# wp133716/test_isaacgym

Measured on AMD Instinct MI355X. Metric: env-steps/sec (whole node), 4096 servo envs; 1/2/4/8-GPU scaling, higher is better.
Workload: dtype f32

## Files before the change

### test_isaacgym_amd/csrc/mg_internal.h

```cpp
#pragma once
#include <hip/hip_runtime.h>
#include <hip/hip_ext.h>
#include <stdint.h>
#include "../../include/migym.h"

#define MG_MAX_CONTACTS 8
#define MG_MAX_LINKS    32
#define MG_MAX_DOFS     32

struct MgStep {
    float h;
    float sub;
    float inv_sub;
    float inv_h;
    float inv_dt;
    float g[3];
    int   substeps, npos, nvel;
    float contact_offset, rest_offset, max_depen, bounce_thresh;
    int   has_ground;
    float n[3];
    float pd;
    float t1[3], t2[3];
    float mu_ground, e_ground;
    float fric_offset;
    float fric_corr;
};

#define MG_TREC_N        (MG_TBODY_F_N + MG_SHAPE_STRIDE + MG_MASS_N)
#define MG_TREC_MASS     (MG_TBODY_F_N + MG_SHAPE_STRIDE)
#ifndef MG_TREC_LDS_MAX
#define MG_TREC_LDS_MAX  (48 * 1024)
#endif

struct MgRigidArgs {
    int          nf;
    int          nf1;
    int          nb;
    const int*   free_ids;
    float*       state;
    const float* mass;
    const int*   body_tmpl;
    const float* tbf;
    const int*   tbi;
    const float* shapes;
    const float* hulls;
    const float* ext;
    float*       cforce;
    const float* trec;
    int          ntb;
    const float* root_src;
    const int*   root_row;
    float*       out_rb;
    float*       out_root;
    const int*   out_body;
    const int*   out_root_row;
    float*       gpatch;
    int          gstride;
    const int*   attr_idx;
    const float* attr;
};

struct MgArticArgs {
    int          na;
    int          nb, nd;
    const int*   artic_i;
    int          aff, ab0, ad0, ads;
    int          out_aff, og0, or0;
    int          tmpl;
    int          nl, ndof;
    int          nbl;
    int          fixed_base;
    int          chain;
    const float* link_f;
    const int*   link_i;
    float*       state;
    const float* mass;
    const int*   body_tmpl;
    const float* tbf;
    float*       dof_pos;
    float*       dof_vel;
    const float* dof_tpos;
    const float* dof_tvel;
    const float* dof_force;
    float*       tpos_w;
    float*       tvel_w;
    float*       force_w;
    const float* dof_props;
    const float* ext;
    float*       cforce;
    const float* uni;
    float*       out_rb;
    float*       out_root;
    float*       out_dof;
    const int*   out_body;
    const int*   out_root_row;
    const int*   attr_idx;
    const float* attr;
    float*       dof_frc;
};

#define MG_ENV_I_N    16
#define MG_ENV_G      16
#define MG_ENV_SLOTS_WIDE 32
#define MG_ENV_MAXF    2
#define MG_ENV_MAXS    4
#define MG_ENV_MAXCT  16
#define MG_ENV_MAXCT_WIDE 48
#define MG_ENV_FREE0  64
// ... 154 lines not shown
```

### test_isaacgym_amd/csrc/mg_rigid.hip

```cpp
#include "mg_internal.h"
#include "mg_math.h"
#include "mg_attractor.h"

#ifdef MG_RIGID1_STAMPS
#define MG_RIGID1_NSTAMP 18
__device__ unsigned long long g_rigid_stamp[4096][MG_RIGID1_NSTAMP];
extern "C" int mg_debug_rigid_stamps(unsigned long long* out, int nwaves) {
    if (nwaves > 4096) nwaves = 4096;
    return hipMemcpyFromSymbol(out, HIP_SYMBOL(g_rigid_stamp), (size_t)nwaves * MG_RIGID1_NSTAMP * 8) == hipSuccess
               ? 0
               : -1;
}
__device__ __forceinline__ unsigned long long rigid_stamp() {
    unsigned long long t;
    __builtin_amdgcn_sched_barrier(0);
    asm volatile("s_memtime %0\n\ts_waitcnt lgkmcnt(0)" : "=s"(t)::"memory");
    __builtin_amdgcn_sched_barrier(0);
    return t;
}
#define RSTAMP(k) do { const unsigned long long t_ = rigid_stamp(); \
    if (threadIdx.x == 0 && blockIdx.x < 4096) g_rigid_stamp[blockIdx.x][k] = t_; } while (0)
#define RUSE(v) asm volatile("" ::"v"(v))
#else
#define RSTAMP(k) do { } while (0)
// ... 523 lines not shown
                const float raw = fmaf(an[a].k2, (pos ? an[a].e2 : 0.0f) - v2, an[a].l2);
                const float nl = clamp_sym(raw, lim);
                const float dl = nl - an[a].l2;
                const bool cl = last && (raw > lim || raw < -lim);
                if (a == 0) c02 = cl; else c12 = cl;
                an[a].l2 = nl;
                V.x = fmaf(-dl, invm, V.x);
                W = pfma(pk2(an[a].I2.x, an[a].I2.y), bc2(dl), W);
                Z.x = fmaf(an[a].I2.z, dl, Z.x);
            }
        }
    };
    const f2 nsub = bc2(-P.inv_sub), psub = bc2(P.sub);
    const int nit = P.npos + P.nvel;
    for (int it = 0; it < P.npos; ++it) {
        const f2 t0 = sep(0) * nsub, t1 = sep(1) * nsub;
        const float tg[4] = {fminf(t0.x, P.max_depen), fminf(t0.y, P.max_depen), fminf(t1.x, P.max_depen),
                             fminf(t1.y, P.max_depen)};
        if (it == 0) {
#pragma unroll
            for (int j = 0; j < 4; ++j) normal(j, tg[j]);
        }
        anchors(true, it == nit - 1);
#pragma unroll
        for (int j = 0; j < 4; ++j) normal(j, tg[j]);
        DV = pfma(V, psub, DV);
        DW = pfma(W, psub, DW);
        DZ = pfma(Z, psub, DZ);
    }
    if (P.nvel > 0) {
        const f2 s01 = sep(0), s23 = sep(1);
        const float sj[4] = {s01.x, s01.y, s23.x, s23.y};
        float tg[4];
#pragma unroll
        for (int j = 0; j < 4; ++j) tg[j] = vel_target(P, sj[j], e, sl[j].vn0);
        for (int it = P.npos; it < nit; ++it) {
#pragma unroll
            for (int j = 0; j < 4; ++j) normal(j, tg[j]);
            anchors(false, it == nit - 1);
#pragma unroll
            for (int j = 0; j < 4; ++j) normal(j, tg[j]);
        }
    }
    v = v3(V.x, V.y, Z.y);
    w = v3(W.x, W.y, Z.x);
    dx = v3(DV.x, DV.y, DZ.y);
    dth = v3(DW.x, DW.y, DZ.x);
}

template <bool PACK, bool ATTR, class B>
__device__ __forceinline__ void rigid_body1(const B& G, const MgStep& P, const float* T, V3& x, Q4& q, V3& v,
                                            V3& w, V3& fsum, float invm, V3 invI, Q4 iq, V3 com, bool has_ext,
                                            V3 fext, V3 text, const float* hulls, float* gp, int gstride,
                                            const float* at) {
    const float lin_damp = T[0], ang_damp = T[1], max_lv = T[2], max_av = T[3], grav_on = T[4];
    float shr[MG_SHAPE_STRIDE];
    const float* sh = T + MG_TBODY_F_N;
    if constexpr (PACK && MG_RIGID1_SHAPE_REGS) {
#pragma unroll
        for (int k = 0; k < 14; ++k) shr[k] = sh[k];
        sh = shr;
    }
    const bool has_shape = P.has_ground && sh[0] >= 0.0f;
    const float rho = sh[13];
    const float h = P.h;
    const float lin_keep = 1.0f - fminf(lin_damp * h, 1.0f);
    const float ang_keep = 1.0f - fminf(ang_damp * h, 1.0f);
    const float max_lv2 = max_lv * max_lv;
    const float max_av2 = max_av * max_av;
    const float mu = 0.5f * (sh[11] + P.mu_ground);
    const float e = 0.5f * (sh[12] + P.e_ground);
    const V3 n0 = v3(P.n[0], P.n[1], P.n[2]);
    GPatch R;
    R.cnt = 0;
    R.dirty = false;
    R.nA = R.aA[0] = R.aA[1] = R.aB[0] = R.aB[1] = v3(0.0f, 0.0f, 0.0f);
    {
        const float clear = G.dn(x) + P.pd;
        const bool far = rho >= 0.0f && clear - rho > P.contact_offset + 1e-3f * (1.0f + fabsf(clear) + rho);
        if (gp && has_shape && !far) {
            float r[MG_FP_N];
#pragma unroll
            for (int k = 0; k < MG_FP_N; ++k) r[k] = gp[(size_t)k * gstride];
            R.cnt = (int)r[0];
            R.nA = v3(r[1], r[2], r[3]);
#pragma unroll
            for (int k = 0; k < 2; ++k) {
                R.aA[k] = v3(r[4 + 6 * k], r[5 + 6 * k], r[6 + 6 * k]);
                R.aB[k] = v3(r[7 + 6 * k], r[8 + 6 * k], r[9 + 6 * k]);
            }
        }
    }

    RUSE(R.cnt); RUSE(R.aA[1].z);
    RSTAMP(2);
    q = qnormalize(q);
    for (int st = 0; st < P.substeps; ++st) {
        const S3 Iw = sym_rdrt(qmat(inertia_frame(q, iq)), invI);
        const V3 xc = com_world(x, q, com);

        if (grav_on != 0.0f) v = vmad(v, v3(P.g[0], P.g[1], P.g[2]), h);
        if (has_ext) {
            v = vmad(v, fext, invm * h);
            w = vmad(w, symmul(Iw, text), h);
        }
        if constexpr (ATTR) {
            if (at) attr_free_body(at, x, q, xc, invm, invI, iq, h, v, w);
        }
        v = vscale(v, lin_keep);
        w = vscale(w, ang_keep);
        {
            float v2 = vdot(v, v);
            if (v2 > max_lv2) v = vscale(v, sqrtf(max_lv2 / v2));
            float w2 = vdot(w, w);
            if (w2 > max_av2) w = vscale(w, sqrtf(max_av2 / w2));
        }

        RUSE(v.x); RUSE(w.z); RUSE(xc.x);
        if (st < 2) RSTAMP(3 + 6 * st);
        NRow sl[4];
        bool on[4];
        V3 cp[4];
#pragma unroll
        for (int j = 0; j < 4; ++j) {
            on[j] = false;
            sl[j].r = v3(0.0f, 0.0f, 0.0f);
            sl[j].s0 = 0.0f;
            cp[j] = v3(0.0f, 0.0f, 0.0f);
        }
        const float clear = G.dn(x) + P.pd;
        const bool far = rho >= 0.0f && clear - rho > P.contact_offset + 1e-3f * (1.0f + fabsf(clear) + rho);
        if (__any(has_shape && !far) && has_shape)
            shape_candidates(G, P, sh, q, x, hulls, [&](int k, V3 p, float sep, float, float) {
// ... 90 lines not shown
                        an[a].l2 = nl;
                        v = G.f2(v, dl, invm);
                        w = fmad3(w, an[a].I2, dl);
                    }
                }
                normals();
                if (pos) {
                    dx = fmad3(dx, v, P.sub);
                    dth = fmad3(dth, w, P.sub);
                }
            }
#pragma unroll
            for (int j = 0; j < 4; ++j) fsum = G.addn(fsum, sl[j].ln);
#pragma unroll
            for (int a = 0; a < 2; ++a) {
                fsum = G.add1(fsum, an[a].l1);
                fsum = G.add2(fsum, an[a].l2);
            }
            const bool one = R.cnt < 2;
            if ((c01 && (c11 || one)) || (c02 && (c12 || one))) R.cnt = 0;
        } else {
            for (int it = 0; it < P.npos; ++it) {
                dx = fmad3(dx, v, P.sub);
                dth = fmad3(dth, w, P.sub);
            }
        }

        RUSE(dx.x); RUSE(dth.z);
        if (st < 2) RSTAMP(7 + 6 * st);
        const V3 xc1 = vadd(xc, dx);
        q = qintegrate(q, dth);
        x = origin_from_com(xc1, q, com);
        RUSE(x.x); RUSE(q.w);
        if (st < 2) RSTAMP(8 + 6 * st);
    }
    if (gp && has_shape) {
        gp[0] = (float)R.cnt;
        if (R.cnt > 0 && R.dirty) {
            const float r[MG_FP_N] = {0.0f, R.nA.x, R.nA.y, R.nA.z,
                                      R.aA[0].x, R.aA[0].y, R.aA[0].z, R.aB[0].x, R.aB[0].y, R.aB[0].z,
                                      R.aA[1].x, R.aA[1].y, R.aA[1].z, R.aB[1].x, R.aB[1].y, R.aB[1].z};
#pragma unroll
            for (int k = 1; k < MG_FP_N; ++k) gp[(size_t)k * gstride] = r[k];
        }
    }
}

#ifndef MG_RIGID1_ROUND_WAVES
#define MG_RIGID1_ROUND_WAVES 2
#endif
#ifndef MG_RIGID1_WIDE_WAVES
#define MG_RIGID1_WIDE_WAVES 3
#endif
template <bool UPZ, bool LDS_T, bool WIDE, bool ATTR>
__global__ void __launch_bounds__(64, UPZ && WIDE ? MG_RIGID1_WIDE_WAVES : (UPZ ? MG_RIGID1_ROUND_WAVES : 2))
k_rigid_step1(MgStep P, MgRigidArgs A) {
    extern __shared__ float s_trec[];
    const int i = (WIDE ? gridDim.x - 1 - blockIdx.x : blockIdx.x) * 64 + threadIdx.x;
    RSTAMP(0);
    const bool live = i < A.nf;
    const int b = A.free_ids ? A.free_ids[live ? i : A.nf - 1] : (live ? i : A.nf - 1);
    const int nb = A.nb;
    const float* Si = A.state + b;
    int si = nb;
    if (A.root_src) {
        const int rr = A.root_row[b];
        if (rr >= 0) {
            Si = A.root_src + (size_t)rr * MG_STATE_N;
            si = 1;
        }
    }
    V3 x = v3(Si[0 * si], Si[1 * si], Si[2 * si]);
    Q4 q = q4(Si[3 * si], Si[4 * si], Si[5 * si], Si[6 * si]);
    V3 v = v3(Si[7 * si], Si[8 * si], Si[9 * si]);
    V3 w = v3(Si[10 * si], Si[11 * si], Si[12 * si]);
    const int tb = A.body_tmpl[b];
#ifdef MG_RIGID1_PREFETCH_OUT
    const bool fout = (A.out_rb || A.out_root) && !WIDE;
    const int pre_ob = fout && A.out_rb ? A.out_body[b] : -1;
    const int pre_or = fout && A.out_root ? A.out_root_row[b] : -1;
#endif
    V3 fext = v3(0.0f, 0.0f, 0.0f), text = v3(0.0f, 0.0f, 0.0f);
    if (A.ext) {
        fext = v3(A.ext[0 * nb + b], A.ext[1 * nb + b], A.ext[2 * nb + b]);
        text = v3(A.ext[3 * nb + b], A.ext[4 * nb + b], A.ext[5 * nb + b]);
    }
    const float* T;
    if constexpr (LDS_T) {
        for (int k = threadIdx.x; k < A.ntb * MG_TREC_N; k += 64) s_trec[k] = A.trec[k];
        __syncthreads();
        T = s_trec + tb * MG_TREC_N;
    } else {
        T = A.trec + tb * MG_TREC_N;
    }
    float mr[11];
    if (T[5] != 0.0f) {
#pragma unroll
        for (int k = 0; k < 11; ++k) mr[k] = T[MG_TREC_MASS + k];
    } else {
#pragma unroll
        for (int k = 0; k < 11; ++k) mr[k] = A.mass[k * nb + b];
    }
    const float invm = mr[0];
    const V3 invI = v3(mr[1], mr[2], mr[3]);
    const Q4 iq = q4(mr[4], mr[5], mr[6], mr[7]);
    const V3 com = v3(mr[8], mr[9], mr[10]);
    V3 fsum = v3(0.0f, 0.0f, 0.0f);
    RUSE(x.x); RUSE(q.w); RUSE(w.z); RUSE(invm); RUSE(com.z); RUSE(T[4]);
    RSTAMP(1);
    float* gp = live && A.gpatch ? A.gpatch + b : nullptr;
    const float* at = nullptr;
    if constexpr (ATTR) {
        const int ai = A.attr_idx[b];
        if (live && ai >= 0) at = A.attr + (size_t)ai * MG_ATTR_N;
    }
    if constexpr (UPZ) {
        rigid_body1<!WIDE, ATTR>(BasisZ{}, P, T, x, q, v, w, fsum, invm, invI, iq, com, A.ext != nullptr, fext, text,
                                 A.hulls, gp, A.gstride, at);
    } else {
        BasisGen G;
        G.n = v3(P.n[0], P.n[1], P.n[2]);
        G.t1 = v3(P.t1[0], P.t1[1], P.t1[2]);
        G.t2 = v3(P.t2[0], P.t2[1], P.t2[2]);
        rigid_body1<!WIDE, ATTR>(G, P, T, x, q, v, w, fsum, invm, invI, iq, com, A.ext != nullptr, fext, text, A.hulls,
                                 gp, A.gstride, at);
    }
    int bo = b;
    asm volatile("" : "+v"(bo));
    if (live) {
        float* So = A.state;
        So[0 * nb + bo] = x.x; So[1 * nb + bo] = x.y; So[2 * nb + bo] = x.z;
        So[3 * nb + bo] = q.x; So[4 * nb + bo] = q.y; So[5 * nb + bo] = q.z; So[6 * nb + bo] = q.w;
        So[7 * nb + bo] = v.x; So[8 * nb + bo] = v.y; So[9 * nb + bo] = v.z;
        So[10 * nb + bo] = w.x; So[11 * nb + bo] = w.y; So[12 * nb + bo] = w.z;
        A.cforce[0 * nb + bo] = fsum.x * P.inv_dt;
        A.cforce[1 * nb + bo] = fsum.y * P.inv_dt;
        A.cforce[2 * nb + bo] = fsum.z * P.inv_dt;
    }
    if ((A.out_rb || A.out_root) && !WIDE) {
        if (live) {
            const float o[MG_STATE_N] = {x.x, x.y, x.z, q.x, q.y, q.z, q.w, v.x, v.y, v.z, w.x, w.y, w.z};
#ifdef MG_RIGID1_PREFETCH_OUT
            const int ob = pre_ob;
            const int rr = pre_or;
#else
            const int ob = A.out_rb ? A.out_body[bo] : -1;
            const int rr = A.out_root ? A.out_root_row[bo] : -1;
#endif
            if (A.out_rb) {
                float* R = A.out_rb + (size_t)ob * MG_STATE_N;
#pragma unroll
                for (int k = 0; k < MG_STATE_N; ++k) R[k] = o[k];
            }
            if (rr >= 0) {
                float* Ro = A.out_root + (size_t)rr * MG_STATE_N;
#pragma unroll
                for (int k = 0; k < MG_STATE_N; ++k) Ro[k] = o[k];
            }
        }
        RSTAMP(15);
#ifdef MG_RIGID1_STAMPS
        asm volatile("s_waitcnt vmcnt(0)" ::: "memory");
        RSTAMP(16);
#endif
    } else if (A.out_rb || A.out_root) {
        __shared__ float s_out[64 * 16];
        __shared__ int s_dst[2][64];
        const int l = threadIdx.x;
        const float o[MG_STATE_N] = {x.x, x.y, x.z, q.x, q.y, q.z, q.w, v.x, v.y, v.z, w.x, w.y, w.z};
#pragma unroll
        for (int k = 0; k < MG_STATE_N; ++k) s_out[l * 16 + k] = o[k];
        s_dst[0][l] = live && A.out_rb ? A.out_body[bo] : -1;
        s_dst[1][l] = live && A.out_root ? A.out_root_row[bo] : -1;
        __syncthreads();
#pragma unroll
        for (int k = 0; k < MG_STATE_N; ++k) {
            const int e = k * 64 + l;
            const int row = e / MG_STATE_N, col = e - row * MG_STATE_N;
            const float val = s_out[row * 16 + col];
            const int d0 = s_dst[0][row], d1 = s_dst[1][row];
            if (d0 >= 0) A.out_rb[(size_t)d0 * MG_STATE_N + col] = val;
            if (d1 >= 0) A.out_root[(size_t)d1 * MG_STATE_N + col] = val;
        }
    }
}

template <bool UPZ, int MAXC, bool MULTI, bool ATTR>
__global__ void __launch_bounds__(64) k_rigid_step(MgStep P, MgRigidArgs A) {
    const int i = blockIdx.x * 64 + threadIdx.x;
    if (i >= A.nf) return;
    const int b = A.free_ids ? A.free_ids[i] : i;
    if constexpr (UPZ) {
        rigid_body<MAXC, MULTI, ATTR>(BasisZ{}, P, A, b);
    } else {
        BasisGen G;
        G.n = v3(P.n[0], P.n[1], P.n[2]);
        G.t1 = v3(P.t1[0], P.t1[1], P.t1[2]);
        G.t2 = v3(P.t2[0], P.t2[1], P.t2[2]);
        rigid_body<MAXC, MULTI, ATTR>(G, P, A, b);
    }
}

}

bool mg_step_is_upz(const MgStep& P) {
    return P.n[0] == 0.0f && P.n[1] == 0.0f && P.n[2] == 1.0f && P.t1[0] == 0.0f && P.t1[1] == 1.0f &&
           P.t1[2] == 0.0f && P.t2[0] == -1.0f && P.t2[1] == 0.0f && P.t2[2] == 0.0f;
}

static int mg_cu_count() {
    static int cus[64] = {0};
    int dev = 0;
    if (hipGetDevice(&dev) != hipSuccess || dev < 0 || dev >= 64) return 256;
    if (cus[dev] <= 0) {
        int n = 0;
        if (hipDeviceGetAttribute(&n, hipDeviceAttributeMultiprocessorCount, dev) != hipSuccess || n <= 0) n = 256;
        cus[dev] = n;
    }
    return cus[dev];
}

hipError_t mg_launch_rigid_step(const MgStep& P, const MgRigidArgs& A, hipStream_t s) {
    if (A.nf <= 0) return hipSuccess;
    const bool upz = mg_step_is_upz(P);
    MgRigidArgs A1 = A, A2 = A;
    A2.root_src = nullptr;
    A2.out_rb = nullptr;
    A2.out_root = nullptr;
    A2.gpatch = nullptr;
    A1.nf = A.nf1;
    A2.nf = A.nf - A.nf1;
    if (A.free_ids) {
        A2.free_ids = A.free_ids + A.nf1;
    } else {
        A2.state = A.state + A.nf1;
        A2.mass = A.mass + A.nf1;
        A2.body_tmpl = A.body_tmpl + A.nf1;
        A2.ext = A.ext ? A.ext + A.nf1 : nullptr;
        A2.cforce = A.cforce + A.nf1;
        A2.attr_idx = A.attr_idx ? A.attr_idx + A.nf1 : nullptr;
    }
    if (A1.nf > 0) {
        const int blocks = (A1.nf + 63) / 64;
        const bool wide = blocks > mg_cu_count() * 4 * (upz ? MG_RIGID1_ROUND_WAVES : 2);
        const size_t lds = (size_t)A.ntb * MG_TREC_N * sizeof(float);
#define MG_K1(U, L) \
    do { \
        if (wide) MG_LAUNCH((k_rigid_step1<U, L, true, false>), dim3(blocks), dim3(64), L ? lds : 0, s, P, A1); \
        else MG_LAUNCH((k_rigid_step1<U, L, false, false>), dim3(blocks), dim3(64), L ? lds : 0, s, P, A1); \
    } while (0)
        if (A1.attr_idx) {
            if (upz && wide) MG_LAUNCH((k_rigid_step1<true, false, true, true>), dim3(blocks), dim3(64), 0, s, P, A1);
            else if (upz) MG_LAUNCH((k_rigid_step1<true, false, false, true>), dim3(blocks), dim3(64), 0, s, P, A1);
            else if (wide) MG_LAUNCH((k_rigid_step1<false, false, true, true>), dim3(blocks), dim3(64), 0, s, P, A1);
            else MG_LAUNCH((k_rigid_step1<false, false, false, true>), dim3(blocks), dim3(64), 0, s, P, A1);
        } else if (lds <= MG_TREC_LDS_MAX) {
            if (upz) MG_K1(true, true);
            else MG_K1(false, true);
        } else {
            if (upz) MG_K1(true, false);
            else MG_K1(false, false);
        }
#undef MG_K1
    }
    if (A2.nf > 0) {
        const int blocks = (A2.nf + 63) / 64;
        if (A2.attr_idx) {
            if (upz) MG_LAUNCH((k_rigid_step<true, MG_MAX_CONTACTS, true, true>), dim3(blocks), dim3(64), 0, s, P, A2);
            else MG_LAUNCH((k_rigid_step<false, MG_MAX_CONTACTS, true, true>), dim3(blocks), dim3(64), 0, s, P, A2);
        } else if (upz) MG_LAUNCH((k_rigid_step<true, MG_MAX_CONTACTS, true, false>), dim3(blocks), dim3(64), 0, s, P, A2);
        else MG_LAUNCH((k_rigid_step<false, MG_MAX_CONTACTS, true, false>), dim3(blocks), dim3(64), 0, s, P, A2);
    }
    return hipGetLastError();
}
```

### test_isaacgym_amd/csrc/migym_capi.cpp

```cpp
#include <hip/hip_runtime.h>

#include <algorithm>
#include <array>
#include <cmath>
#include <cstdio>
#include <cstdarg>
#include <cstring>
#include <string>
#include <map>
#include <vector>

#include "mg_internal.h"
#include "mg_chainlink.h"
#include "mg_attractor.h"

thread_local MgKernelTimer* mg_timer = nullptr;

namespace {

thread_local std::string g_err;

int fail(int code, const char* fmt, ...) __attribute__((format(printf, 2, 3)));
int fail(int code, const char* fmt, ...) {
    char buf[512];
// ... 41 lines not shown
    int attr_count = 0, plain_count = 0;
};

enum AttrClass : char { ATTR_NONE = 0, ATTR_FREE, ATTR_LINK, ATTR_ENV_LINK, ATTR_ENV_FREE, ATTR_PILE };

struct EnvGroup {
    int tmpl, first_link, nl, ndof, floating;
    int wide;
    int max_free;
    int offset, count;
};

}

struct mg_sim {
    int device = 0;
    mg_sim_params params{};
    bool uploaded = false;

    int nenv = 0, na = 0, nb = 0, nd = 0, ntb = 0, ns = 0, nf = 0, nartic = 0, ntl = 0;
    int max_actor_dofs = 0;
    int nf1 = 0;
    int nf_rigid = 0;

    float* d_state = nullptr;
    float* d_mass = nullptr;
    int* d_body_tmpl = nullptr;
    int* d_free_global = nullptr;
    int* d_perm = nullptr;
    float* d_tbf = nullptr;
    float* d_trec = nullptr;
    int* d_tbi = nullptr;
    float* d_shapes = nullptr;
    float* d_hulls = nullptr;
    float* d_shape_obb = nullptr;
    int* d_actor_root = nullptr;
    int* d_body_actor = nullptr;
    int* d_root_row = nullptr;
    bool roots_free = false;
    int fusion = 0;
    const float* pend_root = nullptr;
    const float* pend_tgt[3] = {nullptr, nullptr, nullptr};
    unsigned long long pend_root_cap = 0, pend_tgt_cap[3] = {0, 0, 0}, rb_cap = 0;
    float* bind_root = nullptr;
    float* bind_rb = nullptr;
    float* bind_dof = nullptr;
    long long state_gen = 0, rb_gen = -1, out_gen = -1;
    unsigned long long out_cap = 0;
    long long dof_sgen = 0, dof_gen = -1;
    unsigned long long dof_cap = 0;
    bool step_out_ok = false;
    int* d_slot_global = nullptr;
    int* d_slot_actor = nullptr;
    int last_set_deferred = 0;
    int* d_actor_dof = nullptr;
    float* d_cforce = nullptr;
    float* d_ext = nullptr;
    bool ext_pending = false;

    float* d_dof = nullptr;
    float* d_dof_tgt = nullptr;
    float* d_dof_props = nullptr;
    int* d_artic = nullptr;
    float* d_link_f = nullptr;
    int* d_link_i = nullptr;
    std::vector<ArticGroup> groups;
    int* d_artic_step = nullptr;
    int* d_env = nullptr;
    int* d_pairs = nullptr;
    float* d_fpatch = nullptr;
    float* d_gpatch = nullptr;
    float* d_chain_uni = nullptr;
    unsigned* d_fp_mask = nullptr;
    float* d_env_carry = nullptr;
    int nhull_floats = 0;
    float* d_env_ctab = nullptr;
    int n_coupled = 0;
    std::vector<EnvGroup> env_groups;
    int n_pile = 0;
    int* d_pile_i = nullptr;
    int* d_pile_body = nullptr;
    unsigned* d_pile_pairs = nullptr;
    int* d_pile_slots = nullptr;

    float* d_stage = nullptr;
    size_t stage_n = 0;
    char* h_pin = nullptr;
    size_t h_pin_n = 0;
    hipEvent_t pin_ev = nullptr;
    bool pin_ev_pending = false;
    float* d_host_out = nullptr;
    size_t host_out_n = 0;
    bool has_light = false;
    mg_light light{};
    float* h_stage = nullptr;
    float* d_stage_alias = nullptr;
    size_t h_stage_n = 0;
    float* h_root_in = nullptr;
    float* d_root_in_alias = nullptr;
    hipEvent_t root_ev = nullptr;
    bool root_ev_pending = false;
    bool ho_alias = false;
    const float* ho_written = nullptr;
    long long ho_root_gen = -1, ho_rb_gen = -1, ho_dof_gen = -1;
    int* d_stage_idx = nullptr;
    size_t stage_idx_n = 0;
// ... 187 lines not shown
    HIP_TRY(hipMemcpyAsync(s->d_dof_tgt + (size_t)k * s->nd, src, (size_t)s->nd * sizeof(float),
                           hipMemcpyDeviceToDevice, st));
    return MG_OK;
}

int set_dof_columns(mg_sim* s, const float* src, int src_host, int ncol, float* dst0, float* dst1,
                    const int* idx, int n_idx, hipStream_t st) {
    if (!s || !s->uploaded) return fail(MG_ERR_STATE, "sim has no uploaded model");
    if (s->nd == 0) return MG_OK;
    if (!src) return fail(MG_ERR_ARG, "null source tensor");
    if (idx && n_idx < 0) return fail(MG_ERR_ARG, "negative index count");
    HIP_TRY(hipSetDevice(s->device));
    const float* dsrc;
    const int* didx;
    int rc = stage_src(s, src, src_host, (size_t)s->nd * ncol, idx, n_idx, st, &dsrc, &didx);
    if (rc) return rc;
    float* dst[2] = {dst0, dst1};
    if (idx)
        HIP_TRY(mg_launch_scatter_dofs(dsrc, ncol, s->d_actor_dof, didx, n_idx, s->na, s->max_actor_dofs, dst, st));
    else
        HIP_TRY(mg_launch_scatter_dofs(dsrc, ncol, nullptr, nullptr, s->nd, 0, 1, dst, st));
    return MG_OK;
}

void shape_obb(const float* sh, const float* hulls, float* o) {
    const int t = (int)sh[0];
    for (int k = 0; k < MG_OBB_N; ++k) o[k] = 0.0f;
    if (t == MG_SHAPE_CONVEX && hulls) {
        const float* hv = hulls + (int)sh[2];
        const int nv = (int)hv[0];
        float lo[3], hi[3];
        for (int c = 0; c < 3; ++c) { lo[c] = hv[MG_HULL_HEADER + c]; hi[c] = lo[c]; }
        for (int i = 1; i < nv; ++i)
            for (int c = 0; c < 3; ++c) {
                const float v = hv[MG_HULL_HEADER + 3 * i + c];
                lo[c] = std::min(lo[c], v);
                hi[c] = std::max(hi[c], v);
            }
        for (int c = 0; c < 3; ++c) {
            o[c] = 0.5f * (lo[c] + hi[c]);
            o[3 + c] = 0.5f * (hi[c] - lo[c]);
        }
    } else if (t == MG_SHAPE_BOX) {
        o[3] = sh[1]; o[4] = sh[2]; o[5] = sh[3];
    } else if (t == MG_SHAPE_CAPSULE) {
        o[3] = sh[1] + sh[2]; o[4] = sh[1]; o[5] = sh[1];
    } else {
        o[3] = sh[1]; o[4] = sh[1]; o[5] = sh[1];
    }
}

void free_all(mg_sim* s) {
    void* ptrs[] = {s->d_state, s->d_mass, s->d_body_tmpl, s->d_free_global, s->d_perm, s->d_tbf, s->d_trec, s->d_tbi, s->d_shapes, s->d_hulls, s->d_shape_obb,
                    s->d_actor_root, s->d_root_row, s->d_slot_global, s->d_slot_actor, s->d_body_actor, s->d_actor_dof, s->d_cforce, s->d_ext, s->d_dof, s->d_dof_tgt, s->d_dof_frc,
                    s->d_dof_props, s->d_artic, s->d_artic_step, s->d_env, s->d_pairs, s->d_fpatch, s->d_gpatch, s->d_chain_uni, s->d_fp_mask, s->d_env_carry, s->d_env_ctab, s->d_link_f, s->d_link_i, s->d_stage, s->d_stage_idx, s->d_host_out,
                    s->d_pile_i, s->d_pile_body, s->d_pile_pairs, s->d_pile_slots, s->d_rstate, s->d_rshapes, s->d_env_shape_first, s->d_cams};
    for (void* p : ptrs)
        if (p) (void)hipFree(p);
}

}

extern "C" {

int32_t mg_abi_version(void) { return MG_ABI_VERSION; }
const char* mg_last_error(void) { return g_err.c_str(); }

int32_t mg_device_count(void) {
    int n = 0;
    if (hipGetDeviceCount(&n) != hipSuccess) return 0;
    return n;
}

mg_sim* mg_create_sim(int32_t device, const mg_sim_params* params) {
    if (!params) { fail(MG_ERR_ARG, "null params"); return nullptr; }
    int n = mg_device_count();
    if (n <= 0) { fail(MG_ERR_DEVICE, "no HIP device available (libmigym needs an MI355X)"); return nullptr; }
    if (device < 0 || device >= n) { fail(MG_ERR_DEVICE, "device %d out of range (%d visible)", device, n); return nullptr; }
    if (hipSetDevice(device) != hipSuccess) { fail(MG_ERR_DEVICE, "hipSetDevice(%d) failed", device); return nullptr; }
    mg_sim* s = new mg_sim();
    s->device = device;
    s->params = *params;
    for (int k = 0; k < mg_sim::kRing; ++k) {
        bool ok = hipEventCreate(&s->ring_b[k]) == hipSuccess && hipEventCreate(&s->ring_e[k]) == hipSuccess;
        for (int j = 0; j < mg_sim::kKern && ok; ++j)
            ok = hipEventCreate(&s->kern_b[k][j]) == hipSuccess && hipEventCreate(&s->kern_e[k][j]) == hipSuccess;
        if (!ok) {
            fail(MG_ERR_DEVICE, "hipEventCreate failed");
            mg_destroy_sim(s);
            return nullptr;
        }
    }
    return s;
}

void mg_destroy_sim(mg_sim* s) {
    if (!s) return;
    (void)hipSetDevice(s->device);
    (void)hipDeviceSynchronize();
    free_all(s);
    for (int k = 0; k < mg_sim::kRing; ++k) {
        if (s->ring_b[k]) (void)hipEventDestroy(s->ring_b[k]);
        if (s->ring_e[k]) (void)hipEventDestroy(s->ring_e[k]);
        for (int j = 0; j < mg_sim::kKern; ++j) {
            if (s->kern_b[k][j]) (void)hipEventDestroy(s->kern_b[k][j]);
            if (s->kern_e[k][j]) (void)hipEventDestroy(s->kern_e[k][j]);
        }
// ... 593 lines not shown
        std::vector<float> trec((size_t)s->ntb * MG_TREC_N, 0.0f);
        for (int t = 0; t < s->ntb; ++t) {
            float* r = &trec[(size_t)t * MG_TREC_N];
            std::memcpy(r, m->tmpl_body_f + (size_t)t * MG_TBODY_F_N, MG_TBODY_F_N * sizeof(float));
            const int s0 = m->tmpl_body_i[t * MG_TBODY_I_N + 0], sc = m->tmpl_body_i[t * MG_TBODY_I_N + 1];
            if (sc > 0) {
                const float* sr = m->shapes + (size_t)s0 * MG_SHAPE_STRIDE;
                std::memcpy(r + MG_TBODY_F_N, sr, MG_SHAPE_STRIDE * sizeof(float));
                double ext = -1.0;
                switch ((int)sr[0]) {
                    case MG_SHAPE_SPHERE: ext = sr[1]; break;
                    case MG_SHAPE_BOX: ext = std::sqrt((double)sr[1] * sr[1] + (double)sr[2] * sr[2] + (double)sr[3] * sr[3]); break;
                    case MG_SHAPE_CAPSULE: ext = (double)sr[1] + sr[2]; break;
                    case MG_SHAPE_CONVEX: ext = sr[1]; break;
                    default: break;
                }
                const double po = std::sqrt((double)sr[4] * sr[4] + (double)sr[5] * sr[5] + (double)sr[6] * sr[6]);
                r[MG_TBODY_F_N + 13] = (ext >= 0.0 && std::isfinite(ext + po)) ? (float)((ext + po) * (1.0 + 1e-6)) : -1.0f;
            } else {
                r[MG_TBODY_F_N] = -1.0f;
            }
        }
        std::vector<int> seen(s->ntb, 0), uniform(s->ntb, 1);
        for (int b = 0; b < nb; ++b) {
            if (m->body_kind[b] != MG_BODY_FREE) continue;
            const int t = m->body_tmpl[b];
            const float* mr = m->body_mass + (size_t)b * MG_MASS_N;
            float* r = &trec[(size_t)t * MG_TREC_N];
            if (!seen[t]) {
                std::memcpy(r + MG_TREC_MASS, mr, MG_MASS_N * sizeof(float));
                seen[t] = 1;
            } else if (std::memcmp(r + MG_TREC_MASS, mr, MG_MASS_N * sizeof(float)) != 0) {
                uniform[t] = 0;
            }
        }
        for (int t = 0; t < s->ntb; ++t) trec[(size_t)t * MG_TREC_N + 5] = seen[t] && uniform[t] ? 1.0f : 0.0f;
        HIP_TRY(h2d(s->d_trec, trec.data(), trec.size() * sizeof(float)));
    }
    HIP_TRY(h2d(s->d_shapes, m->shapes, (size_t)s->ns * MG_SHAPE_STRIDE * sizeof(float)));
    if (m->hulls) HIP_TRY(h2d(s->d_hulls, m->hulls, (size_t)m->num_hull_floats * sizeof(float)));
    {
        std::vector<float> obb((size_t)std::max(s->ns, 1) * MG_OBB_N, 0.0f);
        for (int k = 0; k < s->ns; ++k) shape_obb(m->shapes + (size_t)k * MG_SHAPE_STRIDE, m->hulls, &obb[(size_t)k * MG_OBB_N]);
        HIP_TRY(dalloc(&s->d_shape_obb, obb.size()));
        HIP_TRY(h2d(s->d_shape_obb, obb.data(), obb.size() * sizeof(float)));
    }
    HIP_TRY(h2d(s->d_actor_root, root_int.data(), (size_t)na * sizeof(int)));
    {
        std::vector<int> body_actor(nb, -1);
        for (int a = 0; a < na; ++a) body_actor[m->actor_root_body[a]] = a;
        HIP_TRY(dalloc(&s->d_body_actor, (size_t)std::max(nb, 1)));
        HIP_TRY(h2d(s->d_body_actor, body_actor.data(), (size_t)nb * sizeof(int)));
    }
    {
        std::vector<int> row(nb, -1);
        bool ok = s->nf1 == s->nf_rigid && s->nf_rigid == s->nf && s->nartic == 0 && s->n_coupled == 0 &&
                  s->n_pile == 0 && na > 0;
        for (int a = 0; a < na && ok; ++a) {
            const int slot = root_int[a];
            ok = slot >= 0 && slot < s->nf1 && row[slot] < 0;
            if (ok) row[slot] = a;
        }
        s->roots_free = ok;
        HIP_TRY(dalloc(&s->d_root_row, (size_t)std::max(nb, 1)));
        HIP_TRY(h2d(s->d_root_row, row.data(), (size_t)nb * sizeof(int)));
    }
    {
        std::vector<int> slot_actor(nb, -1);
        for (int a = 0; a < na; ++a) slot_actor[root_int[a]] = a;
        HIP_TRY(dalloc(&s->d_slot_global, (size_t)std::max(nb, 1)));
        HIP_TRY(h2d(s->d_slot_global, order.data(), (size_t)nb * sizeof(int)));
        HIP_TRY(dalloc(&s->d_slot_actor, (size_t)std::max(nb, 1)));
        HIP_TRY(h2d(s->d_slot_actor, slot_actor.data(), (size_t)nb * sizeof(int)));
        for (ArticGroup& g : s->groups) {
            g.out_aff = 0;
            if (!g.aff) continue;
            const int* r0 = artic_step.data() + (size_t)g.step_offset * MG_ARTIC_I_N;
            const int G0 = order[r0[0]], A0 = slot_actor[r0[0]];
            bool ok = A0 >= 0;
            for (int k = 0; k < g.step_count && ok; ++k) {
                const int* r = r0 + (size_t)k * MG_ARTIC_I_N;
                ok = slot_actor[r[0]] == A0 + k;
                for (int l = 0; l < g.nl && ok; ++l) ok = order[r[0] + l * r[3]] == G0 + k * g.nl + l;
            }
            if (ok) { g.out_aff = 1; g.out_g0 = G0; g.out_r0 = A0; }
        }
        long long covered = s->nf1 == s->nf_rigid && s->nf_rigid == s->nf ? s->nf1 : -1;
        for (const ArticGroup& g : s->groups) {
            if (covered < 0) break;
            if (g.count == 0) continue;
            if (!(g.chain && g.nl >= 2 && g.nl <= 4) || g.step_count != g.count) covered = -1;
            else covered += (long long)g.step_count * g.nbody;
        }
        s->step_out_ok = s->n_coupled == 0 && s->n_pile == 0 && nb > 0 && covered == nb;
    }
    HIP_TRY(h2d(s->d_actor_dof, m->actor_dof, (size_t)(na + 1) * sizeof(int)));
    HIP_TRY(hipMemset(s->d_cforce, 0, (size_t)nb * 3 * sizeof(float)));
    HIP_TRY(hipMemset(s->d_dof_frc, 0, std::max<size_t>((size_t)nd * 2, 1) * sizeof(float)));
    s->h_actor_dof.assign(m->actor_dof, m->actor_dof + (na > 0 ? na + 1 : 0));
    s->dof_frc_n = 0;
    HIP_TRY(hipMemset(s->d_ext, 0, (size_t)nb * 6 * sizeof(float)));
    if (nd > 0) {
        std::vector<float> ds = to_soa(m->dof_state0, nd, 2);
        HIP_TRY(h2d(s->d_dof, ds.data(), ds.size() * sizeof(float)));
        HIP_TRY(hipMemset(s->d_dof_tgt, 0, (size_t)nd * 3 * sizeof(float)));
        std::vector<float> dp = to_soa(m->dof_props, nd, MG_DOFPROP_N);
        HIP_TRY(h2d(s->d_dof_props, dp.data(), dp.size() * sizeof(float)));
    }
    for (ArticGroup& g : s->groups)
        if (g.uni_mass) chain_uni_dof(m->dof_props, g);
    HIP_TRY(dalloc(&s->d_chain_uni, std::max<size_t>(s->groups.size(), 1) * MG_CHAIN_UNI_N));
    HIP_TRY(chain_uni_upload(s));
    HIP_TRY(h2d(s->d_artic, artic_sorted.data(), artic_sorted.size() * sizeof(int)));
    HIP_TRY(h2d(s->d_artic_step, artic_step.data(), artic_step.size() * sizeof(int)));
    HIP_TRY(h2d(s->d_env, env_flat.data(), env_flat.size() * sizeof(int)));
    HIP_TRY(h2d(s->d_pairs, pairs.data(), pairs.size() * sizeof(int)));
    if (s->n_pile > 0) {
        std::vector<int> flat;
        for (const auto& r : pile_rows) flat.insert(flat.end(), r.begin(), r.end());
        HIP_TRY(dalloc(&s->d_pile_i, flat.size()));
        HIP_TRY(h2d(s->d_pile_i, flat.data(), flat.size() * sizeof(int)));
        HIP_TRY(dalloc(&s->d_pile_body, pile_body.size()));
        HIP_TRY(h2d(s->d_pile_body, pile_body.data(), pile_body.size() * sizeof(int)));
        HIP_TRY(dalloc(&s->d_pile_pairs, std::max<size_t>(pile_pairs.size(), 1)));
        if (!pile_pairs.empty())
            HIP_TRY(h2d(s->d_pile_pairs, pile_pairs.data(), pile_pairs.size() * sizeof(unsigned)));
// ... 133 lines not shown
        }
    }
    for (const EnvGroup& g : s->env_groups) {
        MgEnvArgs A{};
        A.ne = g.count; A.nb = s->nb; A.nd = s->nd;
        A.env_i = s->d_env + (size_t)g.offset * MG_ENV_I_N;
        A.pairs = s->d_pairs;
        A.fpatch = s->d_fpatch;
        A.fp_mask = s->d_fp_mask + (size_t)g.offset * MG_FP_W;
        A.carry = s->d_env_carry + (size_t)g.offset * mg_env_carry_floats();
        A.ctab = s->d_env_ctab + (size_t)g.offset * mg_env_ctab_floats();
        A.nl = g.tmpl >= 0 ? g.nl : 0;
        A.ndof = g.tmpl >= 0 ? g.ndof : 0;
        A.floating = g.tmpl >= 0 ? g.floating : 0;
        A.max_free = g.max_free;
        A.link_f = s->d_link_f + (size_t)(g.tmpl >= 0 ? g.first_link : 0) * MG_LINK_F_N;
        A.link_i = s->d_link_i + (size_t)(g.tmpl >= 0 ? g.first_link : 0) * MG_LINK_I_N;
        A.state = s->d_state; A.mass = s->d_mass; A.body_tmpl = s->d_body_tmpl;
        A.tbf = s->d_tbf; A.tbi = s->d_tbi; A.shapes = s->d_shapes; A.hulls = s->d_hulls;
        A.shape_obb = s->d_shape_obb;
        A.nhull = s->nhull_floats;
        A.nshape = s->ns;
        A.dof_pos = s->d_dof; A.dof_vel = s->d_dof + s->nd;
        A.dof_tpos = s->d_dof_tgt; A.dof_tvel = s->d_dof_tgt + s->nd; A.dof_force = s->d_dof_tgt + 2 * (size_t)s->nd;
        fused_targets(s, A.dof_tpos, A.dof_tvel, A.dof_force, A.tpos_w, A.tvel_w, A.force_w);
        A.dof_props = s->d_dof_props;
        A.ext = s->ext_pending ? s->d_ext : nullptr;
        A.cforce = s->d_cforce;
        A.dof_frc = s->dof_frc_n > 0 ? s->d_dof_frc : nullptr;
        if (s->n_attr_env > 0) {
            A.attr_idx = s->d_attr_idx;
            A.attr = s->d_attr;
        }
        hipError_t e = mg_launch_env_step(P, A, st);
        if (e != hipSuccess) return fail(MG_ERR_DEVICE, "coupled env step launch: %s", hipGetErrorString(e));
    }
    if (s->n_pile > 0) {
        MgPileArgs A{};
        A.ne = s->n_pile; A.nb = s->nb;
        A.pile_i = s->d_pile_i; A.pile_body = s->d_pile_body; A.pairs = s->d_pile_pairs; A.slots = s->d_pile_slots;
        A.state = s->d_state; A.mass = s->d_mass; A.body_tmpl = s->d_body_tmpl; A.tbf = s->d_tbf;
        A.shapes = s->d_shapes; A.hulls = s->d_hulls; A.shape_obb = s->d_shape_obb;
        A.ext = s->ext_pending ? s->d_ext : nullptr;
        A.cforce = s->d_cforce;
        hipError_t e = mg_launch_pile_step(P, A, st);
        if (e != hipSuccess) return fail(MG_ERR_DEVICE, "pile step launch: %s", hipGetErrorString(e));
    }
    if (s->nf_rigid > 0) {
        MgRigidArgs A{};
        A.nf = s->nf_rigid; A.nf1 = s->nf1; A.nb = s->nb; A.free_ids = nullptr;
        A.state = s->d_state; A.mass = s->d_mass; A.body_tmpl = s->d_body_tmpl;
        A.tbf = s->d_tbf; A.tbi = s->d_tbi; A.shapes = s->d_shapes; A.hulls = s->d_hulls;
        A.trec = s->d_trec; A.ntb = s->ntb;
        A.gpatch = s->d_gpatch;
        A.gstride = std::max(s->nf1, 1);
        A.ext = s->ext_pending ? s->d_ext : nullptr;
        A.cforce = s->d_cforce;
        if (s->n_attr_free > 0) {
            A.attr_idx = s->d_attr_idx;
            A.attr = s->d_attr;
        }
        bool reads_root_in = false;
        if (s->pend_root) {
            A.root_src = s->pend_root;
            A.root_row = s->d_root_row;
            reads_root_in = s->pend_root == s->d_root_in_alias;
            s->pend_root = nullptr;
        }
        if (step_out || host_out) {
            A.out_rb = step_out ? s->bind_rb : ho_rb;
            A.out_root = step_out ? s->bind_root : ho_root;
            A.out_body = s->d_slot_global;
            A.out_root_row = s->d_slot_actor;
        }
        HIP_TRY(mg_launch_rigid_step(P, A, st));
        if (reads_root_in) {
            HIP_TRY(hipEventRecord(s->root_ev, st));
            s->root_ev_pending = true;
        }
    }
    if (int rc_ = flush_root(s, st)) return rc_;
    if (s->groups.empty() && s->env_groups.empty())
        for (int k = 0; k < 3; ++k)
            if (int rc_ = flush_tgt(s, k, st)) return rc_;
    for (int k = 0; k < 3; ++k) s->pend_tgt[k] = nullptr;
    s->state_gen++;
    s->dof_sgen++;
    if (host_out) {
        s->ho_written = ho_base;
        s->ho_root_gen = s->state_gen;
        s->ho_rb_gen = s->state_gen;
        s->ho_dof_gen = ho_dof ? s->dof_sgen : -1;
    }
    if (step_out) {
        if (s->bind_root) { s->out_gen = s->state_gen; s->out_cap = step_cid; }
        if (s->bind_rb) { s->rb_gen = s->state_gen; s->rb_cap = step_cid; }
        if (s->bind_dof) { s->dof_gen = s->dof_sgen; s->dof_cap = step_cid; }
    }
    if (s->ext_pending) {
        HIP_TRY(hipMemsetAsync(s->d_ext, 0, (size_t)s->nb * 6 * sizeof(float), st));
        s->ext_pending = false;
    }
    mg_timer = nullptr;
    if (!s->capturing) {
        if (timed) {
            HIP_TRY(hipEventRecord(s->ev_end, st));
// ... 817 lines not shown
```

Baseline: 280.8 million.

## Pack per-slot indices into one record and hoist rigid-step loads ahead of LDS fill

After: 291.6 million, median of 6. 3.9% higher.

```diff
diff --git a/test_isaacgym_amd/csrc/mg_internal.h b/test_isaacgym_amd/csrc/mg_internal.h
--- a/test_isaacgym_amd/csrc/mg_internal.h
+++ b/test_isaacgym_amd/csrc/mg_internal.h
@@ -32,6 +32,10 @@
 #define MG_TREC_LDS_MAX  (48 * 1024)
 #endif
 
+struct alignas(16) MgSlotRec {
+    int root_row, body_tmpl, out_body, out_root_row;
+};
+
 struct MgRigidArgs {
     int          nf;
     int          nf1;
@@ -54,6 +58,7 @@
     float*       out_root;
     const int*   out_body;
     const int*   out_root_row;
+    const MgSlotRec* slot_rec;
     float*       gpatch;
     int          gstride;
     const int*   attr_idx;
diff --git a/test_isaacgym_amd/csrc/mg_rigid.hip b/test_isaacgym_amd/csrc/mg_rigid.hip
--- a/test_isaacgym_amd/csrc/mg_rigid.hip
+++ b/test_isaacgym_amd/csrc/mg_rigid.hip
@@ -599,7 +599,7 @@
 __device__ __forceinline__ void rigid_body1(const B& G, const MgStep& P, const float* T, V3& x, Q4& q, V3& v,
                                             V3& w, V3& fsum, float invm, V3 invI, Q4 iq, V3 com, bool has_ext,
                                             V3 fext, V3 text, const float* hulls, float* gp, int gstride,
-                                            const float* at) {
+                                            const float (&pr)[MG_FP_N], const float* at) {
     const float lin_damp = T[0], ang_damp = T[1], max_lv = T[2], max_av = T[3], grav_on = T[4];
     float shr[MG_SHAPE_STRIDE];
     const float* sh = T + MG_TBODY_F_N;
@@ -625,7 +625,16 @@
     {
         const float clear = G.dn(x) + P.pd;
         const bool far = rho >= 0.0f && clear - rho > P.contact_offset + 1e-3f * (1.0f + fabsf(clear) + rho);
-        if (gp && has_shape && !far) {
+        const bool use = gp && has_shape && !far;
+        if constexpr (PACK) {
+            R.cnt = (int)(use ? pr[0] : 0.0f);
+            R.nA = vsel(use, v3(pr[1], pr[2], pr[3]), R.nA);
+#pragma unroll
+            for (int k = 0; k < 2; ++k) {
+                R.aA[k] = vsel(use, v3(pr[4 + 6 * k], pr[5 + 6 * k], pr[6 + 6 * k]), R.aA[k]);
+                R.aB[k] = vsel(use, v3(pr[7 + 6 * k], pr[8 + 6 * k], pr[9 + 6 * k]), R.aB[k]);
+            }
+        } else if (use) {
             float r[MG_FP_N];
 #pragma unroll
             for (int k = 0; k < MG_FP_N; ++k) r[k] = gp[(size_t)k * gstride];
@@ -822,46 +831,115 @@
 #ifndef MG_RIGID1_WIDE_WAVES
 #define MG_RIGID1_WIDE_WAVES 3
 #endif
-template <bool UPZ, bool LDS_T, bool WIDE, bool ATTR>
+template <bool UPZ, bool LDS_T, bool WIDE, bool ATTR, bool REC = false>
 __global__ void __launch_bounds__(64, UPZ && WIDE ? MG_RIGID1_WIDE_WAVES : (UPZ ? MG_RIGID1_ROUND_WAVES : 2))
 k_rigid_step1(MgStep P, MgRigidArgs A) {
     extern __shared__ float s_trec[];
     const int i = (WIDE ? gridDim.x - 1 - blockIdx.x : blockIdx.x) * 64 + threadIdx.x;
     RSTAMP(0);
+    if constexpr (!WIDE) {
+        asm volatile("" ::"s"(A.nf), "s"(A.free_ids), "s"(A.nb), "s"(A.slot_rec), "s"(A.gpatch), "s"(A.gstride),
+                     "s"(A.trec), "s"(A.ntb), "s"(A.ext), "s"(A.root_src), "s"(A.state), "s"(P.h));
+    }
     const bool live = i < A.nf;
     const int b = A.free_ids ? A.free_ids[live ? i : A.nf - 1] : (live ? i : A.nf - 1);
     const int nb = A.nb;
-    const float* Si = A.state + b;
-    int si = nb;
-    if (A.root_src) {
-        const int rr = A.root_row[b];
-        if (rr >= 0) {
-            Si = A.root_src + (size_t)rr * MG_STATE_N;
-            si = 1;
-        }
-    }
-    V3 x = v3(Si[0 * si], Si[1 * si], Si[2 * si]);
-    Q4 q = q4(Si[3 * si], Si[4 * si], Si[5 * si], Si[6 * si]);
-    V3 v = v3(Si[7 * si], Si[8 * si], Si[9 * si]);
-    V3 w = v3(Si[10 * si], Si[11 * si], Si[12 * si]);
-    const int tb = A.body_tmpl[b];
-#ifdef MG_RIGID1_PREFETCH_OUT
-    const bool fout = (A.out_rb || A.out_root) && !WIDE;
-    const int pre_ob = fout && A.out_rb ? A.out_body[b] : -1;
-    const int pre_or = fout && A.out_root ? A.out_root_row[b] : -1;
-#endif
+    V3 x, v, w;
+    Q4 q;
+    int tb;
     V3 fext = v3(0.0f, 0.0f, 0.0f), text = v3(0.0f, 0.0f, 0.0f);
-    if (A.ext) {
-        fext = v3(A.ext[0 * nb + b], A.ext[1 * nb + b], A.ext[2 * nb + b]);
-        text = v3(A.ext[3 * nb + b], A.ext[4 * nb + b], A.ext[5 * nb + b]);
-    }
     const float* T;
-    if constexpr (LDS_T) {
-        for (int k = threadIdx.x; k < A.ntb * MG_TREC_N; k += 64) s_trec[k] = A.trec[k];
-        __syncthreads();
-        T = s_trec + tb * MG_TREC_N;
+    int pre_ob = -1, pre_or = -1;
+    float pr[MG_FP_N];
+    if constexpr (WIDE) {
+        const float* Si = A.state + b;
+        int si = nb;
+        if (A.root_src) {
+            const int rr = A.root_row[b];
+            if (rr >= 0) {
+                Si = A.root_src + (size_t)rr * MG_STATE_N;
+                si = 1;
+            }
+        }
+        x = v3(Si[0 * si], Si[1 * si], Si[2 * si]);
+        q = q4(Si[3 * si], Si[4 * si], Si[5 * si], Si[6 * si]);
+        v = v3(Si[7 * si], Si[8 * si], Si[9 * si]);
+        w = v3(Si[10 * si], Si[11 * si], Si[12 * si]);
+        tb = A.body_tmpl[b];
+        if (A.ext) {
+            fext = v3(A.ext[0 * nb + b], A.ext[1 * nb + b], A.ext[2 * nb + b]);
+            text = v3(A.ext[3 * nb + b], A.ext[4 * nb + b], A.ext[5 * nb + b]);
+        }
+        if constexpr (LDS_T) {
+            for (int k = threadIdx.x; k < A.ntb * MG_TREC_N; k += 64) s_trec[k] = A.trec[k];
+            __syncthreads();
+            T = s_trec + tb * MG_TREC_N;
+        } else {
+            T = A.trec + tb * MG_TREC_N;
+        }
+#pragma unroll
+        for (int k = 0; k < MG_FP_N; ++k) pr[k] = 0.0f;
     } else {
-        T = A.trec + tb * MG_TREC_N;
+        MgSlotRec rec;
+        if constexpr (REC) {
+            rec = A.slot_rec[b];
+        } else {
+            rec.root_row = A.root_src ? A.root_row[b] : -1;
+            rec.body_tmpl = A.body_tmpl[b];
+            rec.out_body = A.out_rb ? A.out_body[b] : -1;
+            rec.out_root_row = A.out_root ? A.out_root_row[b] : -1;
+        }
+        if (A.gpatch) {
+#pragma unroll
+            for (int k = 0; k < MG_FP_N; ++k) pr[k] = A.gpatch[(size_t)k * A.gstride + b];
+        } else {
+#pragma unroll
+            for (int k = 0; k < MG_FP_N; ++k) pr[k] = 0.0f;
+        }
+        const int nt = A.ntb * MG_TREC_N, l = threadIdx.x;
+        float t0 = 0.0f, t1 = 0.0f;
+        if constexpr (LDS_T) {
+            t0 = A.trec[min(l, nt - 1)];
+            t1 = A.trec[min(l + 64, nt - 1)];
+        }
+        if (A.ext) {
+            fext = v3(A.ext[0 * nb + b], A.ext[1 * nb + b], A.ext[2 * nb + b]);
+            text = v3(A.ext[3 * nb + b], A.ext[4 * nb + b], A.ext[5 * nb + b]);
+        }
+        float s[MG_STATE_N];
+        if (!A.root_src) {
+#pragma unroll
+            for (int k = 0; k < MG_STATE_N; ++k) s[k] = A.state[k * nb + b];
+        }
+        asm volatile("" ::: "memory");
+        if constexpr (LDS_T) {
+            if (l < nt) s_trec[l] = t0;
+            if (l + 64 < nt) s_trec[l + 64] = t1;
+            for (int k = l + 128; k < nt; k += 64) s_trec[k] = A.trec[k];
+            asm volatile("" ::: "memory");
+        }
+        if (!A.root_src) {
+        } else if (rec.root_row >= 0) {
+            const float* Rr = A.root_src + (size_t)rec.root_row * MG_STATE_N;
+#pragma unroll
+            for (int k = 0; k < MG_STATE_N; ++k) s[k] = Rr[k];
+        } else {
+#pragma unroll
+            for (int k = 0; k < MG_STATE_N; ++k) s[k] = A.state[k * nb + b];
+        }
+        x = v3(s[0], s[1], s[2]);
+        q = q4(s[3], s[4], s[5], s[6]);
+        v = v3(s[7], s[8], s[9]);
+        w = v3(s[10], s[11], s[12]);
+        tb = rec.body_tmpl;
+        pre_ob = rec.out_body;
+        pre_or = A.out_root ? rec.out_root_row : -1;
+        if constexpr (LDS_T) {
+            __syncthreads();
+            T = s_trec + tb * MG_TREC_N;
+        } else {
+            T = A.trec + tb * MG_TREC_N;
+        }
     }
     float mr[11];
     if (T[5] != 0.0f) {
@@ -877,6 +955,9 @@
     const V3 com = v3(mr[8], mr[9], mr[10]);
     V3 fsum = v3(0.0f, 0.0f, 0.0f);
     RUSE(x.x); RUSE(q.w); RUSE(w.z); RUSE(invm); RUSE(com.z); RUSE(T[4]);
+    if constexpr (!WIDE) {
+        RUSE(pre_ob); RUSE(pre_or); RUSE(pr[0]); RUSE(pr[MG_FP_N - 1]);
+    }
     RSTAMP(1);
     float* gp = live && A.gpatch ? A.gpatch + b : nullptr;
     const float* at = nullptr;
@@ -886,14 +967,14 @@
     }
     if constexpr (UPZ) {
         rigid_body1<!WIDE, ATTR>(BasisZ{}, P, T, x, q, v, w, fsum, invm, invI, iq, com, A.ext != nullptr, fext, text,
-                                 A.hulls, gp, A.gstride, at);
+                                 A.hulls, gp, A.gstride, pr, at);
     } else {
         BasisGen G;
         G.n = v3(P.n[0], P.n[1], P.n[2]);
         G.t1 = v3(P.t1[0], P.t1[1], P.t1[2]);
         G.t2 = v3(P.t2[0], P.t2[1], P.t2[2]);
         rigid_body1<!WIDE, ATTR>(G, P, T, x, q, v, w, fsum, invm, invI, iq, com, A.ext != nullptr, fext, text, A.hulls,
-                                 gp, A.gstride, at);
+                                 gp, A.gstride, pr, at);
     }
     int bo = b;
     asm volatile("" : "+v"(bo));
@@ -910,13 +991,8 @@
     if ((A.out_rb || A.out_root) && !WIDE) {
         if (live) {
             const float o[MG_STATE_N] = {x.x, x.y, x.z, q.x, q.y, q.z, q.w, v.x, v.y, v.z, w.x, w.y, w.z};
-#ifdef MG_RIGID1_PREFETCH_OUT
             const int ob = pre_ob;
             const int rr = pre_or;
-#else
-            const int ob = A.out_rb ? A.out_body[bo] : -1;
-            const int rr = A.out_root ? A.out_root_row[bo] : -1;
-#endif
             if (A.out_rb) {
                 float* R = A.out_rb + (size_t)ob * MG_STATE_N;
 #pragma unroll
@@ -998,6 +1074,8 @@
     A2.out_rb = nullptr;
     A2.out_root = nullptr;
     A2.gpatch = nullptr;
+    A2.slot_rec = nullptr;
+    if (A.free_ids) A1.slot_rec = nullptr;
     A1.nf = A.nf1;
     A2.nf = A.nf - A.nf1;
     if (A.free_ids) {
@@ -1014,15 +1092,19 @@
         const int blocks = (A1.nf + 63) / 64;
         const bool wide = blocks > mg_cu_count() * 4 * (upz ? MG_RIGID1_ROUND_WAVES : 2);
         const size_t lds = (size_t)A.ntb * MG_TREC_N * sizeof(float);
+        const bool rec = A1.slot_rec != nullptr;
 #define MG_K1(U, L) \
     do { \
         if (wide) MG_LAUNCH((k_rigid_step1<U, L, true, false>), dim3(blocks), dim3(64), L ? lds : 0, s, P, A1); \
+        else if (rec) MG_LAUNCH((k_rigid_step1<U, L, false, false, true>), dim3(blocks), dim3(64), L ? lds : 0, s, P, A1); \
         else MG_LAUNCH((k_rigid_step1<U, L, false, false>), dim3(blocks), dim3(64), L ? lds : 0, s, P, A1); \
     } while (0)
         if (A1.attr_idx) {
             if (upz && wide) MG_LAUNCH((k_rigid_step1<true, false, true, true>), dim3(blocks), dim3(64), 0, s, P, A1);
+            else if (upz && rec) MG_LAUNCH((k_rigid_step1<true, false, false, true, true>), dim3(blocks), dim3(64), 0, s, P, A1);
             else if (upz) MG_LAUNCH((k_rigid_step1<true, false, false, true>), dim3(blocks), dim3(64), 0, s, P, A1);
             else if (wide) MG_LAUNCH((k_rigid_step1<false, false, true, true>), dim3(blocks), dim3(64), 0, s, P, A1);
+            else if (rec) MG_LAUNCH((k_rigid_step1<false, false, false, true, true>), dim3(blocks), dim3(64), 0, s, P, A1);
             else MG_LAUNCH((k_rigid_step1<false, false, false, true>), dim3(blocks), dim3(64), 0, s, P, A1);
         } else if (lds <= MG_TREC_LDS_MAX) {
             if (upz) MG_K1(true, true);
diff --git a/test_isaacgym_amd/csrc/migym_capi.cpp b/test_isaacgym_amd/csrc/migym_capi.cpp
--- a/test_isaacgym_amd/csrc/migym_capi.cpp
+++ b/test_isaacgym_amd/csrc/migym_capi.cpp
@@ -117,6 +117,7 @@
     bool step_out_ok = false;
     int* d_slot_global = nullptr;
     int* d_slot_actor = nullptr;
+    MgSlotRec* d_slot_rec = nullptr;
     int last_set_deferred = 0;
     int* d_actor_dof = nullptr;
     float* d_cforce = nullptr;
@@ -410,7 +411,7 @@
 
 void free_all(mg_sim* s) {
     void* ptrs[] = {s->d_state, s->d_mass, s->d_body_tmpl, s->d_free_global, s->d_perm, s->d_tbf, s->d_trec, s->d_tbi, s->d_shapes, s->d_hulls, s->d_shape_obb,
-                    s->d_actor_root, s->d_root_row, s->d_slot_global, s->d_slot_actor, s->d_body_actor, s->d_actor_dof, s->d_cforce, s->d_ext, s->d_dof, s->d_dof_tgt, s->d_dof_frc,
+                    s->d_actor_root, s->d_root_row, s->d_slot_global, s->d_slot_actor, s->d_slot_rec, s->d_body_actor, s->d_actor_dof, s->d_cforce, s->d_ext, s->d_dof, s->d_dof_tgt, s->d_dof_frc,
                     s->d_dof_props, s->d_artic, s->d_artic_step, s->d_env, s->d_pairs, s->d_fpatch, s->d_gpatch, s->d_chain_uni, s->d_fp_mask, s->d_env_carry, s->d_env_ctab, s->d_link_f, s->d_link_i, s->d_stage, s->d_stage_idx, s->d_host_out,
                     s->d_pile_i, s->d_pile_body, s->d_pile_pairs, s->d_pile_slots, s->d_rstate, s->d_rshapes, s->d_env_shape_first, s->d_cams};
     for (void* p : ptrs)
@@ -1110,6 +1111,7 @@
         HIP_TRY(dalloc(&s->d_body_actor, (size_t)std::max(nb, 1)));
         HIP_TRY(h2d(s->d_body_actor, body_actor.data(), (size_t)nb * sizeof(int)));
     }
+    std::vector<MgSlotRec> slot_rec((size_t)std::max(nb, 1), MgSlotRec{-1, 0, 0, -1});
     {
         std::vector<int> row(nb, -1);
         bool ok = s->nf1 == s->nf_rigid && s->nf_rigid == s->nf && s->nartic == 0 && s->n_coupled == 0 &&
@@ -1122,6 +1124,7 @@
         s->roots_free = ok;
         HIP_TRY(dalloc(&s->d_root_row, (size_t)std::max(nb, 1)));
         HIP_TRY(h2d(s->d_root_row, row.data(), (size_t)nb * sizeof(int)));
+        for (int i = 0; i < nb; ++i) slot_rec[i].root_row = row[i];
     }
     {
         std::vector<int> slot_actor(nb, -1);
@@ -1130,6 +1133,13 @@
         HIP_TRY(h2d(s->d_slot_global, order.data(), (size_t)nb * sizeof(int)));
         HIP_TRY(dalloc(&s->d_slot_actor, (size_t)std::max(nb, 1)));
         HIP_TRY(h2d(s->d_slot_actor, slot_actor.data(), (size_t)nb * sizeof(int)));
+        for (int i = 0; i < nb; ++i) {
+            slot_rec[i].body_tmpl = tmpl_int[i];
+            slot_rec[i].out_body = order[i];
+            slot_rec[i].out_root_row = slot_actor[i];
+        }
+        HIP_TRY(dalloc(&s->d_slot_rec, slot_rec.size()));
+        HIP_TRY(h2d(s->d_slot_rec, slot_rec.data(), (size_t)nb * sizeof(MgSlotRec)));
         for (ArticGroup& g : s->groups) {
             g.out_aff = 0;
             if (!g.aff) continue;
@@ -1369,6 +1379,7 @@
         A.state = s->d_state; A.mass = s->d_mass; A.body_tmpl = s->d_body_tmpl;
         A.tbf = s->d_tbf; A.tbi = s->d_tbi; A.shapes = s->d_shapes; A.hulls = s->d_hulls;
         A.trec = s->d_trec; A.ntb = s->ntb;
+        A.slot_rec = s->d_slot_rec;
         A.gpatch = s->d_gpatch;
         A.gstride = std::max(s->nf1, 1);
         A.ext = s->ext_pending ? s->d_ext : nullptr;
```
